# cudagu/aero-gnn

Hardware: AMD Instinct MI355X
Metric: million edge-updates/sec, 1M-node/6M-edge mesh, 1->8 MI355X (higher is better)
Workload: dtype bf16; 1 GPU; BSMS-MGN 4-scale U-Net train step (fwd+MSE+bwd+allreduce+Adam), 1000000 nodes / 5996000 edges per GPU; model=BiStridedMeshGraphNet(H=128, n_hid=2, processor_size=15, stride=2, concat_trick), mode=train, global_batch=1, parallelism=dp1

## Files before the change

### aero-gnn_amd/aerognn/_lib.py

```python
from __future__ import annotations

import ctypes as C
import os

_HERE = os.path.dirname(os.path.abspath(__file__))
LIB_PATH = os.environ.get("AEROGNN_LIB") or os.path.join(_HERE, "libaerognn.so")

MAX_LIN = 8
MAX_SEG = 3
F32, BF16, F16, F64 = 0, 1, 2, 3
SEG_PLAIN, SEG_GATHER, SEG_SUM, SEG_MEAN = 0, 1, 2, 3
OPT_RESIDENT = 0

vp = C.c_void_p
i32 = C.c_int


class Seg(C.Structure):
    _fields_ = [("kind", i32), ("k", i32), ("ld", i32), ("_pad", i32),
                ("ptr", vp), ("index", vp), ("store", vp)]


ACT = {"relu": 0, "gelu": 1, "silu": 2, "tanh": 3}

# ... 13 lines not shown
class MlpBwdArgs(C.Structure):
    _fields_ = [("rows", i32), ("dtype", i32), ("hidden", i32), ("nlin", i32),
                ("out_dim", i32), ("in_dim", i32), ("use_ln", i32), ("ln_rows", i32),
                ("wtpk", vp * MAX_LIN), ("act", vp * MAX_LIN),
                ("hpre", vp), ("stats", vp), ("ln_g", vp),
                ("g", vp), ("g2", vp), ("gidx", vp),
                ("gpre", vp * MAX_LIN),
                ("din_nseg", i32), ("din_k", i32 * MAX_SEG),
                ("din", vp * MAX_SEG), ("din_resid", i32 * MAX_SEG),
                ("ln_partial", vp), ("tiled", i32), ("gpre_tiled", i32),
                ("mask", vp * MAX_LIN), ("act_fn", i32), ("_pad3", i32), ("pre", vp * MAX_LIN)]


MAX_WGRAD = 8


class WgradDesc(C.Structure):
    _fields_ = [("g", vp), ("x", vp), ("ldg", i32), ("ldx", i32), ("m", i32), ("k", i32), ("rows", i32),
                ("ldw", i32), ("dw_partial", vp), ("db_partial", vp), ("dw", vp), ("db", vp),
                ("g_tiled", i32), ("x_tiled", i32), ("nsplit", i32), ("_pad", i32), ("xidx", vp)]


class WgradBatch(C.Structure):
    _fields_ = [("n", i32), ("_pad", i32), ("d", WgradDesc * MAX_WGRAD)]


class WecArgs(C.Structure):
    _fields_ = [("n", i32), ("e", i32), ("dtype", i32), ("out_dim", i32), ("hid", i32), ("pos_dim", i32),
                ("pos_ld", i32), ("mean", i32),
                ("rowptr", vp), ("src", vp), ("dst", vp), ("perm", vp), ("rowptr_src", vp), ("perm_src", vp),
                ("pos", vp), ("pab", vp), ("tx", vp), ("w1c", vp), ("w2", vp),
                ("w_in", vp), ("w_out", vp), ("out", vp), ("dout", vp), ("gw", vp), ("s_csc", vp), ("dh", vp),
                ("dpa", vp), ("dpb", vp), ("dtx", vp), ("dw_in", vp), ("partial", vp)]


class EdgeBwdArgs(C.Structure):
    _fields_ = [("rows", i32), ("nblk", i32), ("wpk", vp * 4), ("bias", vp * 4), ("ln_g", vp), ("e", vp),
                ("proj", vp), ("src", vp), ("dst", vp), ("g", vp), ("g2", vp), ("de", vp), ("g0", vp),
                ("dw_partial", vp), ("db_partial", vp), ("ln_partial", vp), ("stamps", vp),
                ("a1", vp), ("stats", vp), ("scratch", vp), ("wtpk0", vp),
                ("xk", i32), ("xld", i32)]


class EdgeFwdArgs(C.Structure):
    _fields_ = [("rows", i32), ("nblk", i32), ("wpk", vp * 4), ("bias", vp * 4), ("ln_g", vp), ("ln_b", vp),
                ("e", vp), ("proj", vp), ("src", vp), ("dst", vp), ("out", vp), ("act", vp * 3), ("hpre", vp),
                ("stats", vp)]


class PackDesc(C.Structure):
    _fields_ = [("src", vp), ("dst", vp), ("src_dtype", i32), ("dst_dtype", i32),
                ("rows", i32), ("cols", i32), ("trans", i32), ("ld", i32),
                ("row_off", i32), ("col_off", i32), ("dst_rows", i32), ("dst_cols", i32)]


class F64Seg(C.Structure):
    _fields_ = [("a", vp), ("aidx", vp), ("lda", i32), ("k", i32), ("w", vp), ("ldw", i32), ("transw", i32)]


class F64GemmArgs(C.Structure):
    _fields_ = [("rows", i32), ("n", i32), ("nseg", i32), ("_pad", i32), ("seg", F64Seg * 3), ("bias", vp),
                ("add", vp * 2), ("add_idx", vp * 2), ("add_ld", i32 * 2), ("mask", vp), ("mask_ld", i32),
                ("relu", i32), ("out", vp), ("out_ld", i32), ("mask_act", i32), ("pre_out", vp),
                ("pre_ld", i32), ("_pad3", i32)]


class F64WgradArgs(C.Structure):
    _fields_ = [("rows", i32), ("m", i32), ("k", i32), ("_pad", i32), ("g", vp), ("ldg", i32), ("_pad1", i32),
                ("x", vp), ("ldx", i32), ("_pad2", i32), ("xidx", vp), ("dw", vp), ("ldw", i32), ("_pad3", i32),
                ("db", vp)]


_lib = None

LAUNCHES = ("agn_pack", "agn_mlp_forward", "agn_mlp_backward", "agn_reduce_partials", "agn_wgrad", "agn_colsum",
            "agn_segment_sum", "agn_segment_sum2", "agn_gather_rows", "agn_radix_sort_u64", "agn_row_ptr", "agn_row_ptr_i64",
            "agn_iota_keys", "agn_level_index",
            "agn_exclusive_scan_i32", "agn_pool_sort_keys", "agn_pool_assign", "agn_pool_edge_candidates",
            "agn_pool_edge_sort", "agn_pool_edge_emit", "agn_bfs_distance", "agn_center_seed", "agn_maxdeg_seed",
            "agn_bistride_select", "agn_index_map", "agn_subgraph_edges", "agn_scatter_rows", "agn_wec_forward",
            "agn_wec_backward", "agn_edge_features", "agn_node_features", "agn_normalize", "agn_col_stats", "agn_collate",
            "agn_segment_max", "agn_segment_max_backward", "agn_edge_bwd_fused", "agn_encoder_bwd_fused", "agn_wgrad_reduce",
            "agn_edge_forward32",
            "agn_proj_forward", "agn_proj_backward")


class AeroGNNError(RuntimeError):
    pass


class _Lib:

    def __init__(self, cdll):
        self._cdll = cdll
        for name in LAUNCHES:
            if hasattr(cdll, name):
                setattr(self, name, _timed_launch(getattr(cdll, name), name[4:]))

    def __getattr__(self, name):
        return getattr(self._cdll, name)


def _timed_launch(f, tag):
    from . import core

    def call(*args):
        prof = core.PROF
        if prof is None or core._TIMED_DEPTH:
            return f(*args)
        import torch
        s = torch.cuda.Event(enable_timing=True)
        s.record()
        rc = f(*args)
        e = torch.cuda.Event(enable_timing=True)
        e.record()
        prof.append((tag, None, s, e))
        return rc
    return call


def lib():
    global _lib
    if _lib is None:
        if not os.path.exists(LIB_PATH):
            raise AeroGNNError(
                f"{LIB_PATH} not found: build it with `make -C aero-gnn_amd/csrc` "
                "(or __graft_entry__.build()); the aerognn hot path has no CPU fallback")
        L = C.CDLL(LIB_PATH)
        sig = {
            "agn_version": (i32, []),
            "agn_error_string": (C.c_char_p, [i32]),
            "agn_set_option": (i32, [i32, i32]),
            "agn_packed_bytes": (C.c_size_t, [i32, i32, i32]),
            "agn_pack": (i32, [vp, i32, i32, vp]),
            "agn_mlp_forward": (i32, [C.POINTER(MlpFwdArgs), vp]),
            "agn_mlp_bwd_nwaves": (i32, [i32]),
            "agn_mlp_backward": (i32, [C.POINTER(MlpBwdArgs), vp]),
            "agn_reduce_partials": (i32, [vp, i32, i32, vp, vp]),
            "agn_wgrad_nsplit": (i32, [i32, i32]),
            "agn_wgrad_partial_floats": (C.c_size_t, [i32, i32, i32]),
            "agn_wgrad": (i32, [C.POINTER(WgradBatch), i32, i32, vp]),
            "agn_wgrad_plan": (i32, [C.POINTER(WgradBatch)]),
            "agn_colsum": (i32, [vp, i32, i32, vp, i32, vp, vp]),
            "agn_segment_sum": (i32, [i32, i32, i32, vp, vp, vp, i32, vp, i32, i32, vp]),
            "agn_segment_sum2": (i32, [i32, i32, i32, vp, i32, vp, vp, vp, i32, vp, vp, vp, i32, vp, i32, vp]),
            "agn_gather_rows": (i32, [i32, i32, i32, vp, vp, i32, vp, vp, i32, vp, i32, vp]),
            "agn_segment_max": (i32, [i32, i32, i32, vp, vp, vp, i32, vp, i32, vp, vp]),
            "agn_segment_max_backward": (i32, [i32, i32, i32, vp, vp, i32, vp, i32, vp]),
            "agn_radix_sort_temp_bytes": (C.c_size_t, [i32]),
            "agn_radix_sort_u64": (i32, [vp, vp, i32, i32, vp, vp, vp, vp]),
            "agn_row_ptr": (i32, [vp, i32, i32, vp, vp]),
            "agn_row_ptr_i64": (i32, [vp, i32, i32, vp, vp]),
            "agn_iota_keys": (i32, [i32, vp, vp, vp, vp, vp]),
            "agn_level_index": (i32, [i32, vp, C.c_int64, vp, vp, vp, vp, vp, vp, vp]),
            "agn_scan_temp_bytes": (C.c_size_t, [i32]),
            "agn_exclusive_scan_i32": (i32, [vp, vp, i32, vp, vp, vp]),
            "agn_pool_sort_keys": (i32, [i32, vp, vp, i32, vp, vp, vp]),
            "agn_pool_assign": (i32, [i32, i32, i32, vp, vp, vp, vp, i32, vp, vp, vp, vp, vp]),
            "agn_pool_edge_candidates": (i32, [i32, vp, vp, vp, vp, vp]),
            "agn_pool_edge_sort": (i32, [i32, vp, vp, vp, vp, vp, vp, vp, vp, vp, vp, vp]),
            "agn_pool_edge_emit": (i32, [i32, vp, vp, vp, vp, vp, vp, vp, vp, vp, vp, i32, vp]),
            "agn_bfs_work_ints": (C.c_size_t, [i32]),
            "agn_bfs_distance": (i32, [vp, vp, i32, i32, vp, vp, C.POINTER(i32), vp]),
            "agn_center_seed": (i32, [vp, i32, i32, i32, vp, vp]),
            "agn_maxdeg_seed": (i32, [vp, i32, vp, vp]),
            "agn_compact_work_ints": (C.c_size_t, [i32]),
            "agn_bistride_select": (i32, [vp, i32, vp, C.POINTER(i32), vp, vp]),
            "agn_index_map": (i32, [vp, i32, i32, vp, vp]),
            "agn_subgraph_edges": (i32, [vp, vp, i32, vp, vp, vp, C.POINTER(i32), vp, vp]),
            "agn_scatter_rows": (i32, [i32, i32, i32, vp, vp, i32, vp, i32, vp]),
            "agn_wec_blocks": (i32, [i32]),
            "agn_edge_bwd_blocks": (i32, [i32]),
            "agn_edge_bwd_scratch_bytes": (C.c_size_t, [i32]),
            "agn_edge_features": (i32, [i32, C.c_int64, i32, vp, vp, i32, vp, vp, vp, vp, vp]),
            "agn_normalize": (i32, [i32, i32, vp, i32, vp, vp, vp, i32, i32, vp]),
            "agn_col_stats_temp_bytes": (C.c_size_t, [i32, i32]),
            "agn_col_stats": (i32, [i32, i32, vp, i32, vp, vp, C.c_float, vp, vp]),
            "agn_collate": (i32, [i32, C.c_int64, C.c_int64, vp, vp, vp, vp, vp]),
            "agn_edge_bwd_fused": (i32, [C.POINTER(EdgeBwdArgs), vp]),
            "agn_encoder_bwd_fused": (i32, [C.POINTER(EdgeBwdArgs), vp]),
            "agn_edge_fwd32_blocks": (i32, [i32]),
            "agn_edge_forward32": (i32, [C.POINTER(EdgeFwdArgs), vp]),
            "agn_debug_node32_launches": (C.c_long, []),
            "agn_debug_enc32_launches": (C.c_long, []),
            "agn_debug_dec32_launches": (C.c_long, []),
            "agn_debug_node32_bwd_launches": (C.c_long, []),
            "agn_debug_dec32_bwd_launches": (C.c_long, []),
            "agn_fault_status": (i32, [C.POINTER(i32), i32]),
            "agn_fault_status_async": (i32, [vp, vp]),
            "agn_debug_set_fault": (i32, [i32]),
            "agn_wgrad_reduce": (i32, [C.POINTER(WgradBatch), i32, vp]),
            "agn_proj_forward": (i32, [i32, vp, i32, vp, vp, vp, i32, vp]),
            "agn_proj_backward": (i32, [i32, vp, vp, i32, vp, vp, i32, vp]),
            "agn_wec_forward": (i32, [C.POINTER(WecArgs), vp]),
            "agn_wec_backward": (i32, [C.POINTER(WecArgs), vp]),
            "agn_f64_gemm": (i32, [C.POINTER(F64GemmArgs), vp]),
            "agn_f64_wgrad_scratch_bytes": (C.c_size_t, [C.POINTER(F64WgradArgs)]),
            "agn_f64_wgrad": (i32, [C.POINTER(F64WgradArgs), vp, vp]),
            "agn_f64_layernorm_fwd": (i32, [i32, i32, vp, i32, vp, vp, vp, i32, vp, i32, vp, vp, C.c_double, vp]),
            "agn_f64_layernorm_bwd_scratch_bytes": (C.c_size_t, [i32, i32]),
            "agn_f64_layernorm_bwd": (i32, [i32, i32, vp, i32, vp, i32, vp, vp, vp, vp, i32, vp, vp, vp, vp]),
        }
        for name, (res, args) in sig.items():
            if os.environ.get("AEROGNN_LIB") and name.startswith("agn_debug_") and not hasattr(L, name):
                continue
            f = getattr(L, name)
            f.restype = res
            f.argtypes = args
        _lib = _Lib(L)
    return _lib


def exported_symbols():
    import re
    hdr = os.path.join(_HERE, "..", "..", "include", "aerognn.h")
    txt = open(hdr).read()
    return sorted(set(re.findall(r"\b(agn_[a-z0-9_]+)\s*\(", txt)))


def check(rc: int, what: str = ""):
    if rc != 0:
        msg = lib().agn_error_string(rc).decode()
        raise AeroGNNError(f"aerognn {what} failed: {msg} (code {rc})")


def fault_status(reset=True) -> int:
    v = i32(0)
    check(lib().agn_fault_status(C.byref(v), 1 if reset else 0), "fault_status")
    return int(v.value)


def ptr(t):
    return None if t is None else t.data_ptr()
```

### aero-gnn_amd/aerognn/core.py

```python
from __future__ import annotations

import ctypes as C

import torch

from . import _lib as L
from ._lib import check, ptr


def stream():
    return C.c_void_p(torch.cuda.current_stream().cuda_stream)


PROF = None
_TIMED_DEPTH = 0


class _Timed:
    __slots__ = ("tag", "cost", "s", "on")

    def __init__(self, tag, cost):
        self.tag, self.cost = tag, cost
        self.on = False

# ... 130 lines not shown
                rows, cols = (W.shape[1], W.shape[0]) if tr else (W.shape[0], W.shape[1])
                d = L.PackDesc(W.data_ptr(), base + o, dt_code(W.dtype), code, rows, cols, int(tr),
                               W.stride(0), ro, co, M, K)
                descs.append(d)
                units = ((rows + 31) // 32) * ((cols + 15) // 16) * (2 if code == L.F32 else 1)
                maxthr = max(maxthr, units * 64)
        for key, (n, parts) in self.vecs.items():
            o, nb = offs[key]
            self.views[key] = base + o
            for (v, off) in parts:
                descs.append(L.PackDesc(v.data_ptr(), base + o, dt_code(v.dtype), L.F32, 0, v.numel(), 0, v.stride(0),
                                        0, int(off), 0, n))
                maxthr = max(maxthr, v.numel())
        raw = (L.PackDesc * len(descs))(*descs)
        host = torch.frombuffer(bytearray(bytes(raw)), dtype=torch.uint8)
        self._descs = host.to(device)
        self._ndesc = len(descs)
        self._maxthr = maxthr

    def update(self, dtype, device):
        for key, (M, K, parts) in self.mats.items():
            for p in parts:
                if p[0].dim() != 2 or p[0].stride(1) != 1:
                    raise RuntimeError("aerognn: packed weights need unit column stride (rows may be strided)")
        sig = self._signature(dtype)
        if sig != self._sig:
            self._build(dtype, device)
            self._sig = sig
        check(L.lib().agn_pack(self._descs.data_ptr(), self._ndesc, self._maxthr, stream()), "pack")
        return self

    def __getitem__(self, key):
        return self.views[key]


def mlp_forward(*, rows, dtype, hidden, nlin, out_dim, segs, wpk, bias, out, out_ld=None,
                ln=None, proj=None, src=None, dst=None, resid=None, acts=None, hpre=None, stats=None,
                tag=None, cost=None, act_fn=0):
    a = L.MlpFwdArgs()
    a.rows, a.dtype, a.hidden, a.nlin = rows, dt_code(dtype), hidden, nlin
    a.act_fn = act_fn
    a.out_dim, a.nseg = out_dim, len(segs)
    a.use_ln = 1 if ln is not None else 0
    a.out_ld = out_ld if out_ld is not None else out_dim
    for i, (kind, k, ld, t, idx, store) in enumerate(segs):
        a.seg[i] = L.Seg(kind, k, ld, 0, ptr(t), ptr(idx), ptr(store))
    for i in range(nlin):
        a.wpk[i] = wpk[i]
        a.bias[i] = bias[i]
    if ln is not None:
        a.ln_g, a.ln_b = ln
    a.proj, a.src, a.dst = ptr(proj), ptr(src), ptr(dst)
    a.resid, a.out = ptr(resid), ptr(out)
    if acts is not None:
        for i, t in enumerate(acts):
            a.act[i] = ptr(t)
            a.mask[i] = ptr(_mask_of(t))
            a.pre[i] = ptr(_pre_of(t))
    a.hpre, a.stats = ptr(hpre), ptr(stats)
    a.tiled = int(any(is_tiled(t) for t in list(acts or []) + [hpre]))
    with timed(tag, cost):
        check(L.lib().agn_mlp_forward(C.byref(a), stream()), "mlp_forward")


def proj_kernel_ok(x, H):
    import os
    return (os.environ.get("AEROGNN_PROJ_KERNEL", "1") != "0" and x.dtype == torch.bfloat16 and H == 128
            and x.dim() == 2 and x.shape[1] == 128 and x.stride(1) == 1)


def proj_forward(rows, x, wpk, bias, out, tag=None, cost=None):
    with timed(tag, cost):
        check(L.lib().agn_proj_forward(rows, ptr(x), x.stride(0), wpk, bias, ptr(out), out.stride(0), stream()),
              "proj_forward")


def proj_backward(rows, dps, dpd, wtpk, dx, tag=None, cost=None):
    assert dps.stride(0) == dpd.stride(0)
    with timed(tag, cost):
        check(L.lib().agn_proj_backward(rows, ptr(dps), ptr(dpd), dps.stride(0), wtpk, ptr(dx), dx.stride(0),
                                        stream()), "proj_backward")


def bwd_nblocks(rows):
    return int(L.lib().agn_mlp_bwd_nwaves(int(rows)))


def mlp_backward(*, rows, dtype, hidden, nlin, out_dim, in_dim, wtpk, acts, g, gpre,
                 ln_g=None, hpre=None, stats=None, g2=None, gidx=None, din=(), ln_partial=None,
                 tag=None, cost=None, act_fn=0):
    a = L.MlpBwdArgs()
    a.rows, a.dtype, a.hidden, a.nlin = rows, dt_code(dtype), hidden, nlin
    a.act_fn = act_fn
    a.out_dim, a.in_dim = out_dim, in_dim
    a.use_ln = 1 if ln_g is not None else 0
    for i in range(nlin):
        a.wtpk[i] = wtpk[i]
        a.gpre[i] = ptr(gpre[i]) if gpre[i] is not None else None
    for i, t in enumerate(acts):
        a.act[i] = ptr(t)
        a.mask[i] = ptr(_mask_of(t))
        a.pre[i] = ptr(_pre_of(t))
    a.hpre, a.stats, a.ln_g = ptr(hpre), ptr(stats), ln_g
    a.g, a.g2, a.gidx = ptr(g), ptr(g2), ptr(gidx)
    a.tiled = int(any(is_tiled(t) for t in list(acts or []) + [hpre]))
    a.gpre_tiled = sum(1 << l for l in range(nlin) if is_tiled(gpre[l]))
    a.din_nseg = len(din)
    for i, (k, t, r) in enumerate(din):
        a.din_k[i] = k
        a.din[i] = ptr(t)
        a.din_resid[i] = int(r)
    a.ln_partial = ptr(ln_partial)
    with timed(tag, cost):
        check(L.lib().agn_mlp_backward(C.byref(a), stream()), "mlp_backward")
    return a.ln_rows


CHECK_FAULTS = __import__("os").environ.get("AEROGNN_CHECK_FAULTS", "0") == "1"
STAMPS = None


def fused_edge_train_ok(rows, dtype, hidden, nlin, has_ln):
    import os
    return (os.environ.get("AEROGNN_FUSED_EDGE_BWD", "1") != "0" and dtype == torch.bfloat16 and hidden == 128
            and nlin == 4 and has_ln and rows >= 64 * 1024)


def edge32_ok(dtype, hidden, nlin, has_ln, act=0):
    import os
    return (os.environ.get("AEROGNN_EDGE32", "1") != "0" and dtype == torch.bfloat16 and hidden == 128
            and nlin == 4 and has_ln and act == 0)


def edge_saves_ok():
    import os
    return os.environ.get("AEROGNN_EB_SAVED", "1") != "0"


def edge_forward(*, rows, wpk, bias, ln, e, proj, src, dst, out, a1=None, stats=None, tag=None, cost=None):
    lib = L.lib()
    a = L.EdgeFwdArgs()
    a.rows = int(rows)
    a.nblk = int(lib.agn_edge_fwd32_blocks(int(rows)))
    for i in range(4):
        a.wpk[i] = wpk[i]
        a.bias[i] = bias[i]
    a.ln_g, a.ln_b = ln
    a.e, a.proj, a.src, a.dst, a.out = ptr(e), ptr(proj), ptr(src), ptr(dst), ptr(out)
    a.act[0] = ptr(a1)
    a.stats = ptr(stats)
    with timed(tag, cost):
        check(lib.agn_edge_forward32(C.byref(a), stream()), "edge_forward32")


FAULT_POLL_EVERY = 16
_fault = {"buf": None, "event": None, "n": 0, "dirty": False, "hooked": False, "word": 0}


def _fault_read(block, defer=False):
    st = _fault
    ev = st["event"]
    if ev is not None and (block or ev.query()):
        if block:
            ev.synchronize()
        st["word"] |= int(st["buf"][0])
        st["event"] = None
# ... 322 lines not shown
```

### aero-gnn_amd/aerognn/functions.py

```python
from __future__ import annotations

import ctypes as C

import torch

from . import _lib as L
from ._lib import check, ptr
from . import core as _core
from .core import (Pack, WGrad, alg8d_edge, alg8d_node, with_alg, edge_bwd_fused, fused_edge_train_ok, bwd_nblocks,
                   edge32_ok, edge_saves_ok, edge_forward,
                   cost_edge_bwd_fused,
                   proj_kernel_ok, proj_forward, proj_backward, tiled_empty, relu_mask_empty, colsum_rows, cost_edge_bwd, cost_edge_bwd_cat, cost_edge_fwd,
                   cost_edge_fwd_cat, cost_node_bwd, cost_node_fwd, cost_proj, cost_wec_bwd, cost_wec_fwd, dt_code,
                   timed, gather_rows, mlp_backward, mlp_forward, require_device,
                   scatter_rows, segment_max, segment_max_backward, segment_sum, segment_sum2, stream)


def _c(t):
    return t if t.is_contiguous() else t.contiguous()


def _ln_grads(partial, nblk, M, dtype):
    out = torch.empty(2 * M, dtype=torch.float32, device=partial.device)
    colsum_rows(partial, nblk, 2 * M, out)
    return out[:M].to(dtype), out[M:].to(dtype)


class ChainSpec:

    def __init__(self, linears, ln, hidden, pack: Pack, prefix="", act="relu"):
        if act not in L.ACT:
            raise NotImplementedError(f"aerognn MLP kernels implement activation_fn in {sorted(L.ACT)}, got {act!r}")
        self.act = L.ACT[act]
        self.linears = linears
        self.ln = ln
        self.hidden = hidden
        self.nlin = len(linears)
        self.in_dim = linears[0][0].shape[1]
        self.out_dim = linears[-1][0].shape[0]
        self.tiled_saves = hidden == 128 and (ln is None or self.out_dim == hidden)
        self.p = prefix
        for l, (w, b) in enumerate(linears):
            M, K = w.shape
            pack.matrix(prefix + f"W{l}", M, K, [(w, 0, 0, False)])
            pack.matrix(prefix + f"T{l}", K, M, [(w, 0, 0, True)])
            if b is not None:
                pack.vector(prefix + f"b{l}", M, [(b, 0)])
        if ln is not None:
            pack.vector(prefix + "ln_g", ln[0].numel(), [(ln[0], 0)])
            pack.vector(prefix + "ln_b", ln[1].numel(), [(ln[1], 0)])
        self.pack = pack

    def wpk(self):
        return [self.pack[self.p + f"W{l}"] for l in range(self.nlin)]

    def wtpk(self):
        return [self.pack[self.p + f"T{l}"] for l in range(self.nlin)]

    def biases(self):
        return [self.pack[self.p + f"b{l}"] if self.linears[l][1] is not None else None for l in range(self.nlin)]

    def lnp(self):
        return (self.pack[self.p + "ln_g"], self.pack[self.p + "ln_b"]) if self.ln is not None else None

    def params(self):
        out = []
        for w, b in self.linears:
            out.append(w)
            if b is not None:
                out.append(b)
        if self.ln is not None:
            out += [self.ln[0], self.ln[1]]
        return out

    def check_hidden(self):
        H = self.hidden
        for l, (w, b) in enumerate(self.linears):
            M, K = w.shape
            if l < self.nlin - 1 and M != H:
                raise NotImplementedError(f"aerognn MLP kernels need every hidden width == {H}, got {M}")
            if l > 0 and K != H:
                raise NotImplementedError(f"aerognn MLP kernels need every hidden width == {H}, got {K}")


def _alloc_saves(spec, rows, dtype, dev, train):
    if not train:
        return None, None, None
    emp = tiled_empty if spec.tiled_saves else (lambda r, w, dt, d: torch.empty(r, w, dtype=dt, device=d))
    acts = [emp(rows, spec.hidden, dtype, dev) for _ in range(spec.nlin - 1)]
    for t in acts:
        if spec.act == L.ACT["relu"]:
            t.agn_mask = relu_mask_empty(rows, spec.hidden, dev)
        else:
            t.agn_pre = emp(rows, spec.hidden, dtype, dev)
    hpre = stats = None
# ... 306 lines not shown
                            resid=e, out=e_out, acts=ea, hpre=ehp, stats=est,
                            tag="edge_fwd", cost=with_alg(alg8d_edge(E, N, H, sz), cost_edge_fwd(E, N, H, sz, es.nlin,
                                                                                                train and not fused)))
        else:
            se = (L.SEG_PLAIN, H, e.stride(0), e, None, None)
            ss = (L.SEG_GATHER, H, x.stride(0), x, level.src, None)
            sd = (L.SEG_GATHER, H, x.stride(0), x, level.dst, None)
            mlp_forward(rows=E, dtype=dt, hidden=H, nlin=es.nlin, act_fn=es.act, out_dim=H,
                        segs=[ss, sd, se] if spec.gmp_order else [se, ss, sd],
                        wpk=es.wpk(), bias=es.biases(), ln=es.lnp(), resid=e, out=e_out,
                        acts=ea, hpre=ehp, stats=est,
                        tag="edge_fwd", cost=with_alg(alg8d_edge(E, N, H, x.element_size()),
                                                       cost_edge_fwd_cat(E, N, H, x.element_size(), es.nlin, train)))
        kind = L.SEG_MEAN if spec.aggregation == "mean" else L.SEG_SUM
        agg = torch.empty(N, H, dtype=dt, device=dev) if train else None
        aseg = (kind, H, e_out.stride(0), e_out, level.rowptr, agg)
        mlp_forward(rows=N, dtype=dt, hidden=H, nlin=ns.nlin, act_fn=ns.act, out_dim=H,
                    segs=[(L.SEG_PLAIN, H, x.stride(0), x, None, None), aseg],
                    wpk=ns.wpk(), bias=ns.biases(), ln=ns.lnp(), resid=x, out=x_out,
                    acts=na, hpre=nhp, stats=nst,
                    tag="node_fwd", cost=with_alg(alg8d_node(N, H, x.element_size()),
                                                   cost_node_fwd(E, N, H, x.element_size(),
                                                                 ns.nlin, train)))
        ctx.spec, ctx.level = spec, level
        ctx.saves = (ea, ehp, est, na, nhp, nst, agg)
        ctx.fused, ctx.proj, ctx.esaves = fused, (P if fused and not saved else None), (a1s, sts)
        ctx.save_for_backward(x, e)
        ctx.set_materialize_grads(False)
        return x_out, e_out

    @staticmethod
    def backward(ctx, gx, ge):
        x, e = ctx.saved_tensors
        spec, lv = ctx.spec, ctx.level
        ea, ehp, est, na, nhp, nst, agg = ctx.saves
        es, ns = spec.edge, spec.node
        dt, dev = x.dtype, x.device
        N, E, H = x.shape[0], e.shape[0], spec.H
        gx = _c(gx) if gx is not None else torch.zeros_like(x)
        ge = _c(ge) if ge is not None else None
        gpre_n = _alloc_gpre(ns, N, dt, dev)
        dx = torch.empty_like(x)
        dagg = torch.empty(N, H, dtype=dt, device=dev)
        nb_n = bwd_nblocks(N)
        part_n = torch.empty(nb_n, 2 * H, dtype=torch.float32, device=dev) if ns.ln else None
        nb_n = mlp_backward(rows=N, dtype=dt, hidden=H, nlin=ns.nlin, act_fn=ns.act, out_dim=H, in_dim=2 * H, wtpk=ns.wtpk(),
                     acts=na, g=gx, gpre=gpre_n, ln_g=ns.lnp()[0] if ns.ln else None, hpre=nhp, stats=nst,
                     din=[(H, dx, True), (H, dagg, False)], ln_partial=part_n,
                     tag="node_bwd", cost=with_alg(alg8d_node(N, H, x.element_size(), bwd=True, proj=spec.trick),
                                                   cost_node_bwd(N, H, x.element_size(), ns.nlin)))
        if spec.aggregation == "mean":
            dagg = gather_rows(N, H, None, dagg, torch.empty_like(dagg), cnt_ptr=lv.rowptr)
        fused = ctx.fused
        de = torch.empty_like(e)
        sz = x.element_size()
        if fused:
            g0 = torch.empty(E, H, dtype=dt, device=dev)
            a1s, sts = ctx.esaves
            dW13, db13, part_e, nb_e = edge_bwd_fused(
                rows=E, wpk=es.wpk(), wtpk0=es.wtpk()[0], bias=es.biases(), ln_g=es.lnp()[0], e=e, proj=ctx.proj, src=lv.src, dst=lv.dst,
                g=ge, g2=dagg, de=de, g0=g0, tag="edge_bwd", a1=a1s, stats=sts,
                cost=with_alg(alg8d_edge(E, N, H, sz, bwd=True), cost_edge_bwd_fused(E, N, H, sz, saved=a1s is not None)))
        else:
            nb_e = bwd_nblocks(E)
            part_e = torch.empty(nb_e, 2 * H, dtype=torch.float32, device=dev) if es.ln else None
            gpre_e = _alloc_gpre(es, E, dt, dev, rowmajor=(0,) if spec.trick else ())
            if spec.trick:
                din = [(H, de, True)]
            else:
                dxs = torch.empty(E, H, dtype=dt, device=dev)
                dxd = torch.empty(E, H, dtype=dt, device=dev)
                din = [(H, dxs, False), (H, dxd, False), (H, de, True)] if spec.gmp_order else \
                    [(H, de, True), (H, dxs, False), (H, dxd, False)]
            nb_e = mlp_backward(rows=E, dtype=dt, hidden=H, nlin=es.nlin, act_fn=es.act, out_dim=H, in_dim=es.in_dim,
                                wtpk=es.wtpk(), acts=ea, g=ge, g2=dagg, gidx=lv.dst, gpre=gpre_e,
                                ln_g=es.lnp()[0] if es.ln else None, hpre=ehp, stats=est, din=din, ln_partial=part_e,
                                tag="edge_bwd",
                                cost=with_alg(alg8d_edge(E, N, H, sz, bwd=True),
                                              (cost_edge_bwd if spec.trick else cost_edge_bwd_cat)(E, N, H, sz,
                                                                                                   es.nlin)))
            g0 = gpre_e[0]
        grads_edge = []
        if spec.trick:
            dPs = segment_sum(N, H, lv.rowptr_src, lv.perm_src, g0, torch.empty(N, H, dtype=dt, device=dev))
            dPd = segment_sum(N, H, lv.rowptr, None, g0, torch.empty(N, H, dtype=dt, device=dev))
            if proj_kernel_ok(dx, H):
                s_el = dx.element_size()
                proj_backward(N, dPs, dPd, spec.pack["projT"], dx, tag="proj_bwd",
                              cost=with_alg(alg8d_node(N, H, s_el, bwd=True), (4 * N * H * s_el, 4.0 * N * H * H)))
            else:
                mlp_forward(rows=N, dtype=dt, hidden=H, nlin=1, out_dim=H,
                            segs=[(L.SEG_PLAIN, H, H, dPs, None, None), (L.SEG_PLAIN, H, H, dPd, None, None)],
                            wpk=[spec.pack["projT"]], bias=[None], resid=dx, out=dx)
            eb = spec.eb
            wg = WGrad("wgrad_node")
            if fused:
                dwe = torch.empty(H, H, dtype=torch.float32, device=dev)
                we = WGrad("wgrad_edge")
                we.add(g0, e, dwe)
                we.run()
                eg = [dwe]
                for l in range(3):
                    eg += [dW13[l], db13[l]]
                eg = eg[:1] + [t if t.dtype == p.dtype else t.to(p.dtype) for t, p in zip(eg[1:], es.params()[1:7])]
                eg += list(_ln_grads(part_e, nb_e, H, es.ln[0].dtype))
            else:
                eg = _chain_param_grads(es, gpre_e, e, ea, part_e, nb_e, tag="wgrad_edge")
            dws = torch.empty(H, x.shape[1], dtype=torch.float32, device=dev)
            dwd = torch.empty(H, x.shape[1], dtype=torch.float32, device=dev)
            dbd = torch.empty(H, dtype=torch.float32, device=dev)
            wg.add(dPs, x, dws)
            wg.add(dPd, x, dwd, dbd)
            grads_node = _chain_param_grads(ns, gpre_n, [x, agg], na, part_n, nb_n, wg)
            wg.run()
            if fused and eg[0].dtype != es.linears[0][0].dtype:
                eg[0] = eg[0].to(es.linears[0][0].dtype)
            grads_edge = [eg[0], dws.to(eb.src_lin.dtype), dwd.to(eb.dst_lin.dtype), dbd.to(eb.bias.dtype)] + eg[1:]
            return (dx, de, None, None, None, *grads_edge, *grads_node)
        else:
            segment_sum2(N, H, dx, (lv.rowptr_src, lv.perm_src, dxs), (lv.rowptr, None, dxd), dx)
            xs, xd = (x, lv.src), (x, lv.dst)
            grads_edge = _chain_param_grads(es, gpre_e, [xs, xd, e] if spec.gmp_order else [e, xs, xd],
                                            ea, part_e, nb_e, tag="wgrad_edge")
        grads_node = _chain_param_grads(ns, gpre_n, [x, agg], na, part_n, nb_n, tag="wgrad_node")
        return (dx, de, None, None, None, *grads_edge, *grads_node)


class GradBox:
    __slots__ = ("g", "armed")

    def __init__(self):
        self.g = None
        self.armed = False

    def put(self, g):
        self.g = g if self.g is None else self.g + g

    def take(self):
        if self.armed and self.g is None:
            raise RuntimeError("aerognn: skip gradient missing (autograd order violated)")
        g, self.g = self.g, None
        return g


class SkipFn(torch.autograd.Function):

    @staticmethod
    def forward(ctx, t, box):
        box.armed = True
        ctx.box = box
        return t.view_as(t)

    @staticmethod
    def backward(ctx, g):
        ctx.box.put(g)
        return None, None


class PoolNodeFn(torch.autograd.Function):
    @staticmethod
    def forward(ctx, x, pool, box=None):
        x = _c(x)
        out = torch.empty(pool.nc, x.shape[1], dtype=x.dtype, device=x.device)
        segment_sum(pool.nc, x.shape[1], pool.c2f_ptr, pool.c2f, x, out, mean=True)
        ctx.pool, ctx.box = pool, box
        ctx.n = x.shape[0]
        return out

    @staticmethod
    def backward(ctx, g):
        p = ctx.pool
        g = _c(g)
        add = ctx.box.take() if ctx.box is not None else None
        dx = torch.empty(ctx.n, g.shape[1], dtype=g.dtype, device=g.device)
        gather_rows(ctx.n, g.shape[1], p.f2c, g, dx, cnt_ptr=p.c2f_ptr, add=_c(add) if add is not None else None)
        return dx, None, None
# ... 444 lines not shown
```

### include/aerognn.h

```cpp
#ifndef AEROGNN_H
#define AEROGNN_H
#include <stddef.h>
#include <stdint.h>
#ifdef __cplusplus
extern "C" {
#endif

#define AGN_MAX_LIN 8
#define AGN_MAX_SEG 3

enum { AGN_F32 = 0, AGN_BF16 = 1, AGN_F16 = 2, AGN_F64 = 3 };
enum { AGN_SEG_PLAIN = 0, AGN_SEG_GATHER = 1, AGN_SEG_SUM = 2, AGN_SEG_MEAN = 3 };
enum { AGN_E_ARG = -1, AGN_E_DTYPE = -2, AGN_E_HIDDEN = -3, AGN_E_SHAPE = -4 };
enum { AGN_ACT_RELU = 0, AGN_ACT_GELU = 1, AGN_ACT_SILU = 2, AGN_ACT_TANH = 3 };

typedef struct {
  int kind;
  int k;
  int ld;
  int _pad;
  const void* ptr;
  const int32_t* index;
  void* store;
} agn_seg;
// ... 182 lines not shown
  const int64_t* perm;
  const int32_t* rowptr_src;
  const int32_t* perm_src;
  const float* pos;
  const void* pab;
  const void* tx;
  const float* w1c;
  const float* w2;
  const void* w_in;
  void* w_out;
  void* out;
  const void* dout;
  const void* gw;
  float* s_csc;
  float* dh;
  void* dpa;
  void* dpb;
  void* dtx;
  void* dw_in;
  float* partial;
} agn_wec_args;

int agn_wec_blocks(int n);
int agn_wec_forward(const agn_wec_args* a, void* stream);
int agn_wec_backward(const agn_wec_args* a, void* stream);

typedef struct {
  int rows;
  int nblk;
  const void* wpk[4];
  const float* bias[4];
  const float* ln_g;
  const void* e;
  const void* proj;
  const int32_t* src;
  const int32_t* dst;
  const void* g;
  const void* g2;
  void* de;
  void* g0;
  float* dw_partial;
  float* db_partial;
  float* ln_partial;
  unsigned long long* stamps;
  const void* a1;
  const float* stats;
  void* scratch;
  const void* wtpk0;
  int xk;
  int xld;
} agn_edge_bwd_args;
int agn_edge_bwd_blocks(int rows);
size_t agn_edge_bwd_scratch_bytes(int nblk);
int agn_edge_bwd_fused(const agn_edge_bwd_args* a, void* stream);
int agn_encoder_bwd_fused(const agn_edge_bwd_args* a, void* stream);
#define AGN_FAULT_RING_TIMEOUT 1
int agn_fault_status(int* value, int reset);
int agn_fault_status_async(int* host_pinned, void* stream);
int agn_debug_set_fault(int value);
typedef struct {
  int rows;
  int nblk;
  const void* wpk[4];
  const float* bias[4];
  const float* ln_g;
  const float* ln_b;
  const void* e;
  const void* proj;
  const int32_t* src;
  const int32_t* dst;
  void* out;
  void* act[3];
  void* hpre;
  float* stats;
} agn_edge_fwd_args;
int agn_edge_fwd32_blocks(int rows);
int agn_edge_forward32(const agn_edge_fwd_args* a, void* stream);
int agn_wgrad_reduce(const agn_wgrad_batch* b, int nsplit, void* stream);

int agn_proj_forward(int rows, const void* x, int x_ld, const void* wpk, const float* bias, void* out, int out_ld,
                     void* stream);
int agn_proj_backward(int rows, const void* dps, const void* dpd, int dp_ld, const void* wtpk, void* dx, int dx_ld,
                      void* stream);

int agn_edge_features(int ne, int64_t e_total, int pdim, const int64_t* edge_index, const float* pos, int pos_ld,
                      const int64_t* perm, const float* mean, const float* std, float* out, void* stream);
int agn_normalize(int n, int k, const float* x, int ld, const float* mean, const float* std, float* out, int out_ld,
                  int inverse, void* stream);
size_t agn_col_stats_temp_bytes(int n, int k);
int agn_col_stats(int n, int k, const float* x, int ld, float* mean, float* std, float eps, void* scratch,
                  void* stream);
int agn_collate(int B, int64_t ne, int64_t nn, const int64_t* edge_off, const int64_t* node_off, int64_t* edge_index,
                int64_t* batch, void* stream);

typedef struct {
  const double* a;
  const int32_t* aidx;
  int lda, k;
  const double* w;
  int ldw, transw;
} agn_f64_seg;
typedef struct {
  int rows, n;
  int nseg;
  agn_f64_seg seg[3];
  const double* bias;
  const double* add[2];
  const int32_t* add_idx[2];
  int add_ld[2];
  const double* mask;
  int mask_ld;
  int relu;
  double* out;
  int out_ld;
  int mask_act;
  double* pre_out;
  int pre_ld;
  int _pad3;
} agn_f64_gemm_args;
int agn_f64_gemm(const agn_f64_gemm_args* a, void* stream);
typedef struct {
  int rows, m, k;
  const double* g; int ldg;
  const double* x; int ldx;
  const int32_t* xidx;
  double* dw; int ldw;
  double* db;
} agn_f64_wgrad_args;
size_t agn_f64_wgrad_scratch_bytes(const agn_f64_wgrad_args* a);
int agn_f64_wgrad(const agn_f64_wgrad_args* a, void* scratch, void* stream);
int agn_f64_layernorm_fwd(int rows, int n, const double* x, int ldx, const double* gamma, const double* beta,
                          const double* resid, int ldr, double* y, int ldy, double* mean, double* rstd, double eps,
                          void* stream);
size_t agn_f64_layernorm_bwd_scratch_bytes(int rows, int n);
int agn_f64_layernorm_bwd(int rows, int n, const double* dy, int lddy, const double* x, int ldx, const double* mean,
                          const double* rstd, const double* gamma, double* dx, int lddx, double* dgamma,
                          double* dbeta, void* scratch, void* stream);

#ifdef __cplusplus
}
#endif
#endif
```

Baseline: 786.8 M edge-updates/s.

## Fuse edge-gradient segment sums into projection backward kernel

Adds a new HIP kernel that walks the CSR row pointers per 32-row tile, computes the source- and destination-side segment sums of the edge gradient, writes them out, and immediately applies the projection-transpose GEMM with the residual into dx. This replaces two separate segment_sum launches plus the proj_backward launch in the concat-trick edge backward path. It saves launches and lets the GEMM consume freshly written tiles, prefetching the next tile's row pointers and permutation indices into LDS. The risk is load imbalance from per-tile degree variation and irregular gathers done inside a GEMM-occupancy-constrained kernel.

```diff
diff --git a/aero-gnn_amd/aerognn/_lib.py b/aero-gnn_amd/aerognn/_lib.py
--- a/aero-gnn_amd/aerognn/_lib.py
+++ b/aero-gnn_amd/aerognn/_lib.py
@@ -119,7 +119,7 @@
             "agn_wec_backward", "agn_edge_features", "agn_node_features", "agn_normalize", "agn_col_stats", "agn_collate",
             "agn_segment_max", "agn_segment_max_backward", "agn_edge_bwd_fused", "agn_encoder_bwd_fused", "agn_wgrad_reduce",
             "agn_edge_forward32",
-            "agn_proj_forward", "agn_proj_backward")
+            "agn_proj_forward", "agn_proj_backward", "agn_proj_backward_walk")
 
 
 class AeroGNNError(RuntimeError):
@@ -229,6 +229,7 @@
             "agn_wgrad_reduce": (i32, [C.POINTER(WgradBatch), i32, vp]),
             "agn_proj_forward": (i32, [i32, vp, i32, vp, vp, vp, i32, vp]),
             "agn_proj_backward": (i32, [i32, vp, vp, i32, vp, vp, i32, vp]),
+            "agn_proj_backward_walk": (i32, [i32, vp, i32, vp, vp, vp, vp, vp, vp, i32, vp, i32, vp]),
             "agn_wec_forward": (i32, [C.POINTER(WecArgs), vp]),
             "agn_wec_backward": (i32, [C.POINTER(WecArgs), vp]),
             "agn_f64_gemm": (i32, [C.POINTER(F64GemmArgs), vp]),
@@ -239,7 +240,8 @@
             "agn_f64_layernorm_bwd": (i32, [i32, i32, vp, i32, vp, i32, vp, vp, vp, vp, i32, vp, vp, vp, vp]),
         }
         for name, (res, args) in sig.items():
-            if os.environ.get("AEROGNN_LIB") and name.startswith("agn_debug_") and not hasattr(L, name):
+            if (os.environ.get("AEROGNN_LIB") and not hasattr(L, name)
+                    and (name.startswith("agn_debug_") or name == "agn_proj_backward_walk")):
                 continue
             f = getattr(L, name)
             f.restype = res
diff --git a/aero-gnn_amd/aerognn/core.py b/aero-gnn_amd/aerognn/core.py
--- a/aero-gnn_amd/aerognn/core.py
+++ b/aero-gnn_amd/aerognn/core.py
@@ -236,6 +236,24 @@
                                         stream()), "proj_backward")
 
 
+def proj_walk_ok(x, H):
+    import os
+    return (proj_kernel_ok(x, H) and os.environ.get("AEROGNN_PROJ_WALK", "1") != "0"
+            and hasattr(L.lib(), "agn_proj_backward_walk"))
+
+
+def proj_backward_walk(rows, g0, level, wtpk, dps, dpd, dx, tag="proj_bwd", cost=None):
+    assert dps.stride(0) == dpd.stride(0)
+    perm_src = level.perm_src
+    if g0.shape[0] == 0:
+        g0 = torch.zeros(1, g0.shape[1], dtype=g0.dtype, device=dx.device)
+        perm_src = torch.zeros(4, dtype=torch.int32, device=dx.device)
+    with timed(tag, cost):
+        check(L.lib().agn_proj_backward_walk(rows, ptr(g0), g0.stride(0), ptr(level.rowptr), ptr(level.rowptr_src),
+                                             ptr(perm_src), wtpk, ptr(dps), ptr(dpd), dps.stride(0), ptr(dx),
+                                             dx.stride(0), stream()), "proj_backward_walk")
+
+
 def bwd_nblocks(rows):
     return int(L.lib().agn_mlp_bwd_nwaves(int(rows)))
 
diff --git a/aero-gnn_amd/aerognn/functions.py b/aero-gnn_amd/aerognn/functions.py
--- a/aero-gnn_amd/aerognn/functions.py
+++ b/aero-gnn_amd/aerognn/functions.py
@@ -10,7 +10,8 @@
 from .core import (Pack, WGrad, alg8d_edge, alg8d_node, with_alg, edge_bwd_fused, fused_edge_train_ok, bwd_nblocks,
                    edge32_ok, edge_saves_ok, edge_forward,
                    cost_edge_bwd_fused,
-                   proj_kernel_ok, proj_forward, proj_backward, tiled_empty, relu_mask_empty, colsum_rows, cost_edge_bwd, cost_edge_bwd_cat, cost_edge_fwd,
+                   proj_kernel_ok, proj_forward, proj_backward, proj_walk_ok, proj_backward_walk,
+                   tiled_empty, relu_mask_empty, colsum_rows, cost_edge_bwd, cost_edge_bwd_cat, cost_edge_fwd,
                    cost_edge_fwd_cat, cost_node_bwd, cost_node_fwd, cost_proj, cost_wec_bwd, cost_wec_fwd, dt_code,
                    timed, gather_rows, mlp_backward, mlp_forward, require_device,
                    scatter_rows, segment_max, segment_max_backward, segment_sum, segment_sum2, stream)
@@ -483,16 +484,23 @@
             g0 = gpre_e[0]
         grads_edge = []
         if spec.trick:
-            dPs = segment_sum(N, H, lv.rowptr_src, lv.perm_src, g0, torch.empty(N, H, dtype=dt, device=dev))
-            dPd = segment_sum(N, H, lv.rowptr, None, g0, torch.empty(N, H, dtype=dt, device=dev))
-            if proj_kernel_ok(dx, H):
-                s_el = dx.element_size()
-                proj_backward(N, dPs, dPd, spec.pack["projT"], dx, tag="proj_bwd",
-                              cost=with_alg(alg8d_node(N, H, s_el, bwd=True), (4 * N * H * s_el, 4.0 * N * H * H)))
+            s_el = dx.element_size()
+            if proj_walk_ok(dx, H) and g0.dtype == dx.dtype:
+                dPs = torch.empty(N, H, dtype=dt, device=dev)
+                dPd = torch.empty(N, H, dtype=dt, device=dev)
+                proj_backward_walk(N, g0, lv, spec.pack["projT"], dPs, dPd, dx, tag="proj_bwd",
+                                   cost=with_alg(alg8d_node(N, H, s_el, bwd=True),
+                                                 (E * H * s_el + 4 * N * H * s_el, 4.0 * N * H * H)))
             else:
-                mlp_forward(rows=N, dtype=dt, hidden=H, nlin=1, out_dim=H,
-                            segs=[(L.SEG_PLAIN, H, H, dPs, None, None), (L.SEG_PLAIN, H, H, dPd, None, None)],
-                            wpk=[spec.pack["projT"]], bias=[None], resid=dx, out=dx)
+                dPs = segment_sum(N, H, lv.rowptr_src, lv.perm_src, g0, torch.empty(N, H, dtype=dt, device=dev))
+                dPd = segment_sum(N, H, lv.rowptr, None, g0, torch.empty(N, H, dtype=dt, device=dev))
+                if proj_kernel_ok(dx, H):
+                    proj_backward(N, dPs, dPd, spec.pack["projT"], dx, tag="proj_bwd",
+                                  cost=with_alg(alg8d_node(N, H, s_el, bwd=True), (4 * N * H * s_el, 4.0 * N * H * H)))
+                else:
+                    mlp_forward(rows=N, dtype=dt, hidden=H, nlin=1, out_dim=H,
+                                segs=[(L.SEG_PLAIN, H, H, dPs, None, None), (L.SEG_PLAIN, H, H, dPd, None, None)],
+                                wpk=[spec.pack["projT"]], bias=[None], resid=dx, out=dx)
             eb = spec.eb
             wg = WGrad("wgrad_node")
             if fused:
diff --git a/aero-gnn_amd/csrc/projwalk.hip b/aero-gnn_amd/csrc/projwalk.hip
--- /dev/null
+++ b/aero-gnn_amd/csrc/projwalk.hip
@@ -0,0 +1,204 @@
+#include "tile32.hpp"
+#include "aerognn.h"
+
+using namespace agn;
+using namespace agn::t32;
+
+namespace {
+
+#ifndef AGN_PW_NW
+#define AGN_PW_NW 8
+#endif
+#ifndef AGN_PW_NQ
+#define AGN_PW_NQ 6
+#endif
+constexpr int NW = AGN_PW_NW;
+constexpr int NQ = AGN_PW_NQ;
+constexpr int PF = 2;
+constexpr int KU = 2 * NU;
+constexpr int PW_UNITS = NT * KU * 64;
+constexpr int NIR = 8;
+constexpr int ICAP = 64 * NIR;
+
+struct Smem {
+  uint4 w[PW_UNITS];
+  uint4 stg[NW][8][H / 8 + STG_PAD];
+  int rp[NW][2][64];
+  int idx[NW][ICAP];
+};
+static_assert(sizeof(Smem) <= 160 * 1024, "LDS budget");
+
+AGN_DEV void walk_tile(const bf16* __restrict__ G, int g_ld, const int* rpd, const int* rps,
+                       const int32_t* __restrict__ perm, const int* lidx, int tsb, bf16* dpd, bf16* dps, int out_ld,
+                       int tile, int rows, int lane) {
+  const int g = lane >> 4, k = lane & 15;
+  const bf16* gk = G + 8 * k;
+#pragma unroll 1
+  for (int bt = 0; bt < 4; ++bt) {
+    int beg[4], end[4];
+#pragma unroll
+    for (int t = 0; t < 4; ++t) {
+      const int nl = 8 * bt + 4 * (t & 1) + g;
+      const int* rp = t < 2 ? rpd : rps;
+      beg[t] = rp[nl];
+      end[t] = rp[nl + 1];
+    }
+    float sum[4][8];
+#pragma unroll
+    for (int t = 0; t < 4; ++t)
+#pragma unroll
+      for (int e = 0; e < 8; ++e) sum[t][e] = 0.f;
+    const int steps = max(max(end[0] - beg[0], end[1] - beg[1]), max(end[2] - beg[2], end[3] - beg[3]));
+#pragma unroll 1
+    for (int j = 0; j < steps; j += NQ) {
+      int e[2][NQ];
+#pragma unroll
+      for (int n = 0; n < 2; ++n)
+#pragma unroll
+        for (int q = 0; q < NQ; ++q) {
+          const int jj = beg[2 + n] + j + q;
+          e[n][q] = 0;
+          if (jj < end[2 + n]) e[n][q] = jj - tsb < ICAP ? lidx[jj - tsb] : perm[jj];
+        }
+      uint4 r[4][NQ];
+#pragma unroll
+      for (int t = 0; t < 4; ++t)
+#pragma unroll
+        for (int q = 0; q < NQ; ++q) {
+          const int jj = beg[t] + j + q;
+          if (jj < end[t]) r[t][q] = *reinterpret_cast<const uint4*>(gk + (size_t)(t < 2 ? jj : e[t - 2][q]) * g_ld);
+        }
+#pragma unroll
+      for (int t = 0; t < 4; ++t)
+#pragma unroll
+        for (int q = 0; q < NQ; ++q)
+          if (beg[t] + j + q < end[t]) {
+            const u32x4 x = __builtin_bit_cast(u32x4, r[t][q]);
+#pragma unroll
+            for (int d = 0; d < 4; ++d) {
+              sum[t][2 * d] += lo_bf16(x[d]);
+              sum[t][2 * d + 1] += hi_bf16(x[d]);
+            }
+          }
+    }
+#pragma unroll
+    for (int t = 0; t < 4; ++t) {
+      const float(&sv)[8] = sum[t];
+      const u32x4 pk = {pack2(sv[0], sv[1]), pack2(sv[2], sv[3]), pack2(sv[4], sv[5]), pack2(sv[6], sv[7])};
+      const int row = tile * 32 + 8 * bt + 4 * (t & 1) + g;
+      if (row < rows) *reinterpret_cast<u32x4*>((t < 2 ? dpd : dps) + (size_t)row * out_ld + 8 * k) = pk;
+    }
+  }
+}
+
+__global__ __launch_bounds__(64 * NW) void proj_walk_kernel(int rows, const bf16* __restrict__ g0, int g0_ld,
+                                                            const int32_t* __restrict__ rowptr,
+                                                            const int32_t* __restrict__ rowptr_src,
+                                                            const int32_t* __restrict__ perm_src,
+                                                            const uint4* __restrict__ wpk, bf16* dps, bf16* dpd,
+                                                            int dp_ld, bf16* dx, int dx_ld) {
+  __shared__ Smem sm;
+  for (int i = threadIdx.x; i < PW_UNITS; i += 64 * NW) sm.w[i] = wpk[i];
+  __syncthreads();
+  const int lane0 = threadIdx.x & 63;
+  const int w = __builtin_amdgcn_readfirstlane(threadIdx.x >> 6);
+  const int ntiles = (rows + 31) / 32;
+  const Walk walk(ntiles, w, NW);
+  int* rpd = sm.rp[w][0];
+  int* rps = sm.rp[w][1];
+  int* lidx = sm.idx[w];
+  auto tile_rp = [&](const int32_t* p, int t) { return p[min(t * 32 + min(lane0, 32), rows)]; };
+  auto idx_issue = [&](int (&ir)[NIR], int lane) {
+    const int b = rps[0], e = rps[32];
+#pragma unroll
+    for (int i = 0; i < NIR; ++i) {
+      const int pj = b + lane + 64 * i;
+      ir[i] = pj < e ? perm_src[pj] : 0;
+    }
+  };
+  auto idx_park = [&](const int (&ir)[NIR], int lane) {
+#pragma unroll
+    for (int i = 0; i < NIR; ++i) lidx[lane + 64 * i] = ir[i];
+  };
+  if (walk.first < walk.end) {
+    rpd[lane0] = tile_rp(rowptr, walk.first);
+    rps[lane0] = tile_rp(rowptr_src, walk.first);
+    int ir[NIR];
+    idx_issue(ir, lane0);
+    idx_park(ir, lane0);
+  }
+  for (int tile = walk.first; tile < walk.end; tile += walk.step) {
+    cbarrier();
+    const int lane = opaque_v(lane0);
+    const bool more = tile + walk.step < walk.end;
+    const int nt = more ? tile + walk.step : tile;
+    const int nrd = tile_rp(rowptr, nt), nrs = tile_rp(rowptr_src, nt);
+    walk_tile(g0, g0_ld, rpd, rps, perm_src, lidx, rps[0], dpd, dps, dp_ld, tile, rows, lane);
+    if (more) {
+      rpd[lane] = nrd;
+      rps[lane] = nrs;
+    }
+    __builtin_amdgcn_fence(__ATOMIC_RELEASE, "workgroup");
+    __builtin_amdgcn_wave_barrier();
+    __builtin_amdgcn_fence(__ATOMIC_ACQUIRE, "workgroup");
+    const int nvalid = rows - tile * 32;
+    const size_t t0 = (size_t)tile * 32;
+    bf16* dxt = dx + t0 * dx_ld;
+    uint4 raws[NR / 8], rawd[NR / 8], rawx[NR / 8];
+    int ir[NIR];
+    tile_load_issue<H / 8>(raws, dps + t0 * dp_ld, nvalid, lane, dp_ld / 8);
+    if constexpr (NW <= 8) {
+      tile_load_issue<H / 8>(rawd, dpd + t0 * dp_ld, nvalid, lane, dp_ld / 8);
+      tile_load_issue<H / 8>(rawx, dxt, nvalid, lane, dx_ld / 8);
+      if (more) idx_issue(ir, lane);
+    }
+    f32x16 acc[NT];
+#pragma unroll
+    for (int t = 0; t < NT; ++t)
+#pragma unroll
+      for (int r = 0; r < 16; ++r) acc[t][r] = 0.f;
+    uint4 mine[NR / 8];
+    BOp<bf16, NR> b;
+    tile_load_finish<H / 8>(mine, raws, sm.stg[w], lane);
+    b.set_w(mine);
+    if constexpr (NW > 8) tile_load_issue<H / 8>(rawd, dpd + t0 * dp_ld, nvalid, lane, dp_ld / 8);
+    gemm_stream<PF>(acc, b, sm.w, KU, 0, 0, lane);
+    tile_load_finish<H / 8>(mine, rawd, sm.stg[w], lane);
+    b.set_w(mine);
+    if constexpr (NW > 8) {
+      tile_load_issue<H / 8>(rawx, dxt, nvalid, lane, dx_ld / 8);
+      if (more) idx_issue(ir, lane);
+    }
+    gemm_stream<PF>(acc, b, sm.w, KU, 0, NU, lane);
+    if (more) idx_park(ir, lane);
+    tile_load_finish<H / 8>(mine, rawx, sm.stg[w], lane);
+    const int h = lane >> 5;
+    uint4 ob[NR / 8];
+#pragma unroll
+    for (int i = 0; i < NR / 8; ++i) {
+      float v8[8], r8[8];
+      acc_get8(v8, acc, i);
+      unpack8_w(r8, mine[i]);
+#pragma unroll
+      for (int e = 0; e < 8; ++e) v8[e] = round_t<bf16>(v8[e]) + r8[e];
+      ob[i] = pack8_w(v8, h);
+    }
+    tile_store_chunks<H / 8>(ob, dxt, nvalid, sm.stg[w], lane, dx_ld / 8);
+  }
+}
+
+}
+
+extern "C" int agn_proj_backward_walk(int rows, const void* g0, int g0_ld, const int32_t* rowptr,
+                                      const int32_t* rowptr_src, const int32_t* perm_src, const void* wtpk, void* dps,
+                                      void* dpd, int dp_ld, void* dx, int dx_ld, void* stream) {
+  if (rows < 0 || !g0 || !rowptr || !rowptr_src || !perm_src || !wtpk || !dps || !dpd || !dx || g0_ld % 8 ||
+      dp_ld % 8 || dx_ld % 8 || g0_ld < H || dp_ld < H || dx_ld < H || !al16(g0) || !al16(wtpk) || !al16(dps) ||
+      !al16(dpd) || !al16(dx) || dps == g0 || dpd == g0 || dps == dpd)
+    return AGN_E_ARG;
+  if (rows == 0) return 0;
+  hipLaunchKernelGGL(proj_walk_kernel, dim3(tile_blocks((rows + 31) / 32, NW)), dim3(64 * NW), 0, (hipStream_t)stream,
+                     rows, (const bf16*)g0, g0_ld, rowptr, rowptr_src, perm_src, (const uint4*)wtpk, (bf16*)dps,
+                     (bf16*)dpd, dp_ld, (bf16*)dx, dx_ld);
+  return launch_status();
+}
diff --git a/include/aerognn.h b/include/aerognn.h
--- a/include/aerognn.h
+++ b/include/aerognn.h
@@ -288,6 +288,9 @@
                      void* stream);
 int agn_proj_backward(int rows, const void* dps, const void* dpd, int dp_ld, const void* wtpk, void* dx, int dx_ld,
                       void* stream);
+int agn_proj_backward_walk(int rows, const void* g0, int g0_ld, const int32_t* rowptr, const int32_t* rowptr_src,
+                           const int32_t* perm_src, const void* wtpk, void* dps, void* dpd, int dp_ld, void* dx,
+                           int dx_ld, void* stream);
 
 int agn_edge_features(int ne, int64_t e_total, int pdim, const int64_t* edge_index, const float* pos, int pos_ld,
                       const int64_t* perm, const float* mean, const float* std, float* out, void* stream);
```

New measurement: 789.9 M edge-updates/s, median of 5. Within noise of the previous version (+0.4%).
